# hby1320/pytorch_object_detection

Measured on AMD Instinct MI355X. Metric: images/sec HISFCOS-R50 640x640 inference, higher is better.
Workload: dtype f32

## Files before the change

### include/fcosdet.h

```cpp
#ifndef FCOSDET_H_
#define FCOSDET_H_

#include <stdint.h>

#ifdef __cplusplus
extern "C" {
#endif

#define FD_OK 0
#define FD_E_INVAL (-1)
#define FD_E_UNSUPPORTED (-2)
#define FD_E_LAUNCH (-3)

#define FD_MAX_SEG 8

#define FD_ACT_NONE 0
#define FD_ACT_RELU 1
#define FD_ACT_SILU 2
#define FD_ACT_EXP 3
#define FD_ACT_SIGMOID 4

typedef void* fd_stream_t;

typedef struct fd_segs {
// ... 229 lines not shown
                                     int32_t H, int32_t W, const float* mean3, const float* std3, fd_stream_t stream);
int32_t fd_jitter_l_sums(const uint8_t* const* images_dev, int32_t* recs_dev, uint64_t* sums_dev, int32_t N,
                         int64_t max_pixels, fd_stream_t stream);
int32_t fd_color_jitter_u8(const uint8_t* x, int32_t h, int32_t w, uint8_t* y, const int32_t* rec_dev, fd_stream_t stream);
int32_t fd_rotate_u8(const uint8_t* x, int32_t h, int32_t w, uint8_t* y, const int32_t* fixed6, fd_stream_t stream);

int64_t fd_groupnorm_workspace_bytes(const fd_segs* segs, int32_t G);
int32_t fd_groupnorm_act_nhwc(const float* x, int32_t x_cs, int32_t x_co, const float* gamma, const float* beta,
                              float* y, int32_t y_cs, int32_t y_co, int32_t C, int32_t G, float eps, int32_t act,
                              const fd_segs* segs, void* workspace, fd_stream_t stream);

int64_t fd_groupnorm_bwd_workspace_bytes(const fd_segs* segs, int32_t C);
int32_t fd_groupnorm_act_bwd_nhwc(const float* x, int32_t x_cs, int32_t x_co, const float* dy, int32_t dy_cs,
                                  int32_t dy_co, const float* gamma, const float* beta, float* dx, int32_t dx_cs,
                                  int32_t dx_co, float* dgamma, float* dbeta, int32_t C, int32_t G, float eps,
                                  int32_t act, const fd_segs* segs, const void* fwd_workspace, void* workspace,
                                  fd_stream_t stream);

int64_t fd_se_workspace_bytes(int32_t N, int32_t HW, int32_t C);
int32_t fd_se_scale_nhwc(const float* x, int32_t x_cs, int32_t x_co, const float* w1, const float* b1,
                         const float* w2, const float* b2, float* y, int32_t y_cs, int32_t y_co, int32_t N,
                         int32_t HW, int32_t C, int32_t Cr, void* workspace, fd_stream_t stream);

int64_t fd_se_bwd_workspace_bytes(int32_t N, int32_t HW, int32_t C);
int32_t fd_se_scale_bwd_nhwc(const float* x, int32_t x_cs, int32_t x_co, const float* dy, int32_t dy_cs, int32_t dy_co,
                             const float* w1, const float* b1, const float* w2, const float* b2, float* dx, int32_t dx_cs,
                             int32_t dx_co, float* dw1, float* db1, float* dw2, float* db2, int32_t N, int32_t HW, int32_t C,
                             int32_t Cr, const void* fwd_workspace, void* workspace, fd_stream_t stream);

int32_t fd_act_nhwc(const float* x, int32_t x_cs, int32_t x_co, float* y, int32_t y_cs, int32_t y_co, int64_t rows, int32_t C,
                    int32_t act, float param, fd_stream_t stream);
int32_t fd_act_bwd_nhwc(const float* x, int32_t x_cs, int32_t x_co, const float* dy, int32_t dy_cs, int32_t dy_co, float* dx,
                        int32_t dx_cs, int32_t dx_co, int64_t rows, int32_t C, int32_t act, float param, fd_stream_t stream);
int32_t fd_act_bwd_nhwc_h(const void* x, int32_t x_cs, int32_t x_co, const void* dy, int32_t dy_cs, int32_t dy_co, void* dx,
                          int32_t dx_cs, int32_t dx_co, int64_t rows, int32_t C, int32_t act, float param, fd_stream_t stream);

int32_t fd_maxpool_bwd_nhwc(const float* x, int32_t x_cs, int32_t x_co, const float* dy, int32_t dy_cs, int32_t dy_co, float* dx,
                            int32_t dx_cs, int32_t dx_co, int32_t N, int32_t H, int32_t W, int32_t C, int32_t k, int32_t s,
                            int32_t pad, fd_stream_t stream);
int32_t fd_upsample2x_bwd_nhwc(const float* dy, int32_t dy_cs, int32_t dy_co, float* dx, int32_t dx_cs, int32_t dx_co, int32_t N,
                               int32_t H, int32_t W, int32_t C, fd_stream_t stream);

int32_t fd_groupnorm_from_rowstats(const float* rowstats, int32_t C, int32_t G, float eps, const float* gamma, const float* beta,
                                   const fd_segs* segs, void* workspace, float* coef, fd_stream_t stream);
int32_t fd_groupnorm_apply_nhwc(const float* x, int32_t x_cs, int32_t x_co, const float* gamma, const float* beta, float* y,
                                int32_t y_cs, int32_t y_co, int32_t C, int32_t G, float eps, int32_t act, const fd_segs* segs,
// ... 114 lines not shown
```

### pytorch_object_detection_amd/_lib.py

```python
from __future__ import annotations

import ctypes as C
import os

FD_MAX_SEG = 8
ACT_NONE, ACT_RELU, ACT_SILU, ACT_EXP, ACT_SIGMOID = 0, 1, 2, 3, 4
CONV_GENERIC, CONV_STEM = 0, 1
PREC_F32, PREC_F16X3, PREC_F16 = 0, 1, 2
TILES = {1: (128, 128), 2: (128, 64), 3: (64, 128), 4: (64, 64), 5: (128, 32), 6: (128, 96),
         7: (128, 128), 8: (128, 64), 9: (64, 128),
         10: (256, 128), 11: (256, 128),
         12: (128, 96),
         13: (128, 128),
         15: (64, 64)}
PATCH_TILE = 13
WAVE_TILE = 15
WINO_TILE = 14
WINO4_TILE = 16
NARROW_TILE = 17
F16K64_TILE = 18

_HERE = os.path.dirname(os.path.abspath(__file__))
LIB_PATH = os.environ.get("FD_LIB") or os.path.join(_HERE, "csrc", "libfcosdet_hip.so")

# ... 125 lines not shown
    "fd_resize_u8": (_I, [_P, _I, _I, _P, _I, _I, _P]),
    "fd_resize_collate_u8_nhwc4": (_I, [_P, _P, _P, _P, _I, _I, _I, C.POINTER(_F), C.POINTER(_F), _P]),
    "fd_boxes_scale_batch": (_I, [_P, _P, _P, _I, _I, _I, _I, _P]),
    "fd_augment_resize_collate_u8": (_I, [_P, _P, _P, _I, _I, _I, C.POINTER(_F), C.POINTER(_F), _P]),
    "fd_jitter_l_sums": (_I, [_P, _P, _P, _I, _L, _P]),
    "fd_color_jitter_u8": (_I, [_P, _I, _I, _P, _P, _P]),
    "fd_rotate_u8": (_I, [_P, _I, _I, _P, C.POINTER(_I), _P]),
    "fd_dwconv_dilated_wgrad_workspace_bytes": (_L, [C.POINTER(Segs), _I, _I]),
    "fd_dwconv_dilated_bwd_weight_nhwc": (_I, [_P, _I, _I, _P, _I, _I, _P, _I, _I, _I, _P, _I, C.POINTER(Segs), _P, _P]),
    "fd_dwconv3x3_wgrad_workspace_bytes": (_L, [C.POINTER(Segs), _I]),
    "fd_dwconv3x3_bwd_weight_nhwc": (_I, [_P, _I, _I, _P, _I, _I, _P, _I, _P, _I, C.POINTER(Segs), _P, _P]),
    "fd_groupnorm_workspace_bytes": (_L, [C.POINTER(Segs), _I]),
    "fd_groupnorm_act_nhwc": (_I, [_P, _I, _I, _P, _P, _P, _I, _I, _I, _I, _F, _I, C.POINTER(Segs), _P, _P]),
    "fd_groupnorm_from_rowstats": (_I, [_P, _I, _I, _F, _P, _P, C.POINTER(Segs), _P, _P, _P]),
    "fd_groupnorm_apply_nhwc": (_I, [_P, _I, _I, _P, _P, _P, _I, _I, _I, _I, _F, _I, C.POINTER(Segs), _P, _P]),
    "fd_groupnorm_stats_nhwc": (_I, [_P, _I, _I, _I, _I, _F, _P, _P, C.POINTER(Segs), _P, _P, _P]),
    "fd_coef_apply_nhwc": (_I, [_P, _I, _I, _P, _P, _I, _P, _I, _I, _I, _I, C.POINTER(Segs), _P]),
    "fd_dwconv3x3_gn_nhwc": (_I, [_P, _I, _I, _P, _P, _I, _P, _I, _I, _I, _P, _I, C.POINTER(Segs), _P]),
    "fd_groupnorm_bwd_workspace_bytes": (_L, [C.POINTER(Segs), _I]),
    "fd_groupnorm_act_bwd_nhwc": (_I, [_P, _I, _I, _P, _I, _I, _P, _P, _P, _I, _I, _P, _P, _I, _I, _F, _I, C.POINTER(Segs), _P, _P,
                                       _P]),
    "fd_se_workspace_bytes": (_L, [_I, _I, _I]),
    "fd_se_scale_nhwc": (_I, [_P, _I, _I, _P, _P, _P, _P, _P, _I, _I, _I, _I, _I, _I, _P, _P]),
    "fd_se_bwd_workspace_bytes": (_L, [_I, _I, _I]),
    "fd_se_scale_bwd_nhwc": (_I, [_P, _I, _I, _P, _I, _I, _P, _P, _P, _P, _P, _I, _I, _P, _P, _P, _P, _I, _I, _I, _I, _P, _P, _P]),
    "fd_act_nhwc": (_I, [_P, _I, _I, _P, _I, _I, _L, _I, _I, _F, _P]),
    "fd_act_bwd_nhwc": (_I, [_P, _I, _I, _P, _I, _I, _P, _I, _I, _L, _I, _I, _F, _P]),
    "fd_act_bwd_nhwc_h": (_I, [_P, _I, _I, _P, _I, _I, _P, _I, _I, _L, _I, _I, _F, _P]),
    "fd_maxpool_bwd_nhwc": (_I, [_P, _I, _I, _P, _I, _I, _P, _I, _I, _I, _I, _I, _I, _I, _I, _I, _P]),
    "fd_upsample2x_bwd_nhwc": (_I, [_P, _I, _I, _P, _I, _I, _I, _I, _I, _I, _P]),
    "fd_batchnorm_update_running": (_I, [_P, _L, _I, _F, _F, _P, _P, _P]),
    "fd_batchnorm_update_running_dev": (_I, [_P, _P, _I, _F, _F, _P, _P, _P]),
    "fd_batchnorm_sync_fwd_nhwc": (_I, [_P, _I, _I, _P, _P, _P, _I, _I, _L, _I, _F, _I, _I, _P, _D, _P, _P]),
    "fd_batchnorm_sync_bwd_nhwc": (_I, [_P, _I, _I, _P, _I, _I, _P, _P, _P, _I, _I, _P, _P, _L, _I, _F, _I, _I, _P, _D, _P, _P, _P]),
    "fd_fcos_decode": (_I, [_P, _I, _I, _P, _I, _I, _P, _I, _I, _I, C.POINTER(Segs), C.POINTER(_I), _P, _P, _P, _P]),
    "fd_topk_workspace_bytes": (_L, [_I, _I, _I]),
    "fd_fcos_topk": (_I, [_P, _P, _P, _I, _I, _I, _P, _P, _P, _P, _P, _P]),
    "fd_nms_workspace_bytes": (_L, [_I, _I]),
    "fd_batched_nms": (_I, [_P, _P, _P, _I, _I, _F, _D, _P, _P, _P, _P, _P, _P, _P]),
    "fd_box_nms_plus1": (_I, [_P, _P, _P, _I, _I, _F, _I, _P, _P, _P]),
    "fd_pairwise_iou": (_I, [_P, _P, _I, _I, _I, _P, _P]),
    "fd_clip_boxes": (_I, [_P, _L, _I, _I, _P]),
    "fd_pack_detections": (_I, [_P, _P, _P, _P, _I, _I, _P, _P]),
    "fd_unpack_detections": (_I, [_P, _I, _I, _P, _P, _P, _P, _P]),
    "fd_ltrb_iou_loss_fwd": (_I, [_P, _P, _P, _I, _I, _I, _P, _P, _P]),
    "fd_ltrb_iou_loss_bwd": (_I, [_P, _P, _P, _P, _I, _I, _I, _P, _P]),
# ... 39 lines not shown
```

### pytorch_object_detection_amd/csrc/fd_layers.hip

```cpp
#include "fd_common.h"

#define FD_GRID_CAP 16384

static inline unsigned grid_for(long work, int block) {
    long g = (work + block - 1) / block;
    if (g > FD_GRID_CAP) g = FD_GRID_CAP;
    if (g < 1) g = 1;
    return (unsigned)g;
}

__global__ __launch_bounds__(256) void nchw3_to_nhwc4_kernel(const float* __restrict__ x, float4* __restrict__ y,
                                                              int HW, long total) {
    for (long i = (long)blockIdx.x * 256 + threadIdx.x; i < total; i += (long)gridDim.x * 256) {
        int pi;
        const long n = fd_div(i, HW, pi);
        const long p = pi;
        const float* b = x + n * 3 * HW + p;
        y[i] = make_float4(b[0], b[HW], b[2 * (long)HW], 0.f);
    }
}

extern "C" int32_t fd_nchw3_to_nhwc4(const float* x, float* y, int32_t N, int32_t H, int32_t W, fd_stream_t stream) {
    FD_REQUIRE(x && y && N >= 1 && H >= 1 && W >= 1, FD_E_INVAL, "fd_nchw3_to_nhwc4: bad argument");
    FD_REQUIRE(((uintptr_t)y & 15) == 0, FD_E_INVAL, "fd_nchw3_to_nhwc4: y not 16-byte aligned");
// ... 332 lines not shown
__device__ __forceinline__ void seg_decode(const fd_segs& sg, long m, int& H, int& W, long& img_row0, int& h, int& w) {
    int s = 0;
#pragma unroll
    for (int t = 1; t < FD_MAX_SEG; ++t)
        if (t < sg.nseg && m >= sg.m_start[t]) s = t;
    H = sg.H[s]; W = sg.W[s];
    const long local = m - sg.m_start[s];
    const int hw = H * W;
    int rem;
    const long n = fd_div(local, hw, rem);
    h = rem / W; w = rem - h * W;
    img_row0 = sg.m_start[s] + n * hw;
}

struct StripTab {
    fd_segs s;
    long strip_start[FD_MAX_SEG + 1];
    int spr[FD_MAX_SEG];
};

__device__ __forceinline__ float dw_quad_xor1(float v) { return __builtin_bit_cast(float, __builtin_amdgcn_mov_dpp(__builtin_bit_cast(int, v), 0xB1, 0xF, 0xF, true)); }
__device__ __forceinline__ float dw_quad_xor2(float v) { return __builtin_bit_cast(float, __builtin_amdgcn_mov_dpp(__builtin_bit_cast(int, v), 0x4E, 0xF, 0xF, true)); }

template <int S, bool FUSE = false>
__global__ __launch_bounds__(256) void dwconv3x3_strip_kernel(const float* __restrict__ x, int x_cs, int x_co,
                                                               const float* __restrict__ wt, const float* __restrict__ scale,
                                                               const float* __restrict__ shift, float* __restrict__ y, int y_cs,
                                                               int y_co, int C, int act, StripTab tab, long total,
                                                               const float* __restrict__ in_coef = nullptr, int in_act = 0,
                                                               float* __restrict__ gn_stats = nullptr, int gn_G = 1) {
    const int C4 = C >> 2;
    for (long i = (long)blockIdx.x * 256 + threadIdx.x; i < total; i += (long)gridDim.x * 256) {
        int q;
        const long t = fd_div(i, C4, q);
        int s = 0;
#pragma unroll
        for (int k = 1; k < FD_MAX_SEG; ++k)
            if (k < tab.s.nseg && t >= tab.strip_start[k]) s = k;
        const int H = tab.s.H[s], W = tab.s.W[s], spr = tab.spr[s];
        const long local = t - tab.strip_start[s];
        const int per_img = H * spr;
        int rem;
        const long n = fd_div(local, per_img, rem);
        const int h = rem / spr, w0 = (rem - h * spr) * S;
        const long r0 = (long)tab.s.m_start[s] + n * H * W;
        float4 ca = make_float4(1.f, 1.f, 1.f, 1.f), cb = make_float4(0.f, 0.f, 0.f, 0.f);
        const float act_lo = (FUSE && in_act == FD_ACT_RELU) ? 0.f : -INFINITY;
        if (FUSE && in_coef) {
            const float* cp = in_coef + ((long)(s * tab.s.batch + (int)n) * 2) * C + 4 * q;
            ca = *reinterpret_cast<const float4*>(cp);
            cb = *reinterpret_cast<const float4*>(cp + C);
        }
        float4 acc[S];
#pragma unroll
        for (int j = 0; j < S; ++j) acc[j] = make_float4(0.f, 0.f, 0.f, 0.f);
#pragma unroll
        for (int r = 0; r < 3; ++r) {
            const int hi = h + r - 1;
            if ((unsigned)hi >= (unsigned)H) continue;
            float4 u[S + 2];
#pragma unroll
            for (int c = 0; c < S + 2; ++c) {
                const int wi = w0 + c - 1;
                u[c] = (unsigned)wi < (unsigned)W ? *reinterpret_cast<const float4*>(x + (r0 + (long)hi * W + wi) * x_cs + x_co + 4 * q)
                                                  : make_float4(0.f, 0.f, 0.f, 0.f);
            }
            if (FUSE && in_coef) {
#pragma unroll
                for (int c = 0; c < S + 2; ++c) {
                    float4 t = make_float4(fmaf(u[c].x, ca.x, cb.x), fmaf(u[c].y, ca.y, cb.y), fmaf(u[c].z, ca.z, cb.z), fmaf(u[c].w, ca.w, cb.w));
                    t.x = fmaxf(t.x, act_lo); t.y = fmaxf(t.y, act_lo); t.z = fmaxf(t.z, act_lo); t.w = fmaxf(t.w, act_lo);
                    if (in_act == FD_ACT_SILU) {
                        t.x *= __builtin_amdgcn_rcpf(1.0f + __expf(-t.x)); t.y *= __builtin_amdgcn_rcpf(1.0f + __expf(-t.y));
                        t.z *= __builtin_amdgcn_rcpf(1.0f + __expf(-t.z)); t.w *= __builtin_amdgcn_rcpf(1.0f + __expf(-t.w));
                    }
                    const bool inb = (unsigned)(w0 + c - 1) < (unsigned)W;
                    u[c] = inb ? t : make_float4(0.f, 0.f, 0.f, 0.f);
                }
            }
#pragma unroll
            for (int c = 0; c < 3; ++c) {
                const float4 k = *reinterpret_cast<const float4*>(wt + (r * 3 + c) * C + 4 * q);
#pragma unroll
                for (int j = 0; j < S; ++j) {
                    if ((unsigned)(w0 + j + c - 1) < (unsigned)W) {
                        acc[j].x = fmaf(u[j + c].x, k.x, acc[j].x); acc[j].y = fmaf(u[j + c].y, k.y, acc[j].y);
                        acc[j].z = fmaf(u[j + c].z, k.z, acc[j].z); acc[j].w = fmaf(u[j + c].w, k.w, acc[j].w);
                    }
                }
            }
        }
        float4 sc = make_float4(1.f, 1.f, 1.f, 1.f), sf = make_float4(0.f, 0.f, 0.f, 0.f);
        if (scale) sc = *reinterpret_cast<const float4*>(scale + 4 * q);
        if (shift) sf = *reinterpret_cast<const float4*>(shift + 4 * q);
#pragma unroll
        for (int j = 0; j < S; ++j) {
            if (w0 + j >= W) break;
            float4 o;
            o = fd_act4(make_float4(acc[j].x * sc.x + sf.x, acc[j].y * sc.y + sf.y, acc[j].z * sc.z + sf.z, acc[j].w * sc.w + sf.w), act, 0.f);
            const long mo = r0 + (long)h * W + w0 + j;
            *reinterpret_cast<float4*>(y + mo * y_cs + y_co + 4 * q) = o;
            if (FUSE && gn_stats) {
                float s1 = (o.x + o.y) + (o.z + o.w), s2 = (o.x * o.x + o.y * o.y) + (o.z * o.z + o.w * o.w);
                const int cgq = (C / gn_G) >> 2;
                if (cgq > 1) { s1 += dw_quad_xor1(s1); s2 += dw_quad_xor1(s2); }
                if (cgq > 2) { s1 += dw_quad_xor2(s1); s2 += dw_quad_xor2(s2); }
                if (cgq > 4) { s1 += __shfl_xor(s1, 4); s2 += __shfl_xor(s2, 4); }
                if ((q & (cgq - 1)) == 0) reinterpret_cast<float2*>(gn_stats)[mo * gn_G + (4 * q) / (C / gn_G)] = make_float2(s1, s2);
            }
        }
    }
}

extern "C" int32_t fd_dwconv3x3_nhwc(const float* x, int32_t x_cs, int32_t x_co, const float* w, const float* scale,
                                     const float* shift, float* y, int32_t y_cs, int32_t y_co, int32_t C, int32_t act,
                                     const fd_segs* segs, fd_stream_t stream) {
    FD_REQUIRE(fd_segs_ok(segs), FD_E_INVAL, "fd_dwconv3x3: bad segment table");
    FD_REQUIRE(view_ok(x, x_cs, x_co, C) && view_ok(y, y_cs, y_co, C) && w && ((uintptr_t)w & 15) == 0, FD_E_INVAL,
               "fd_dwconv3x3: channel views must be 4-aligned (C=%d)", C);
    StripTab tab; tab.s = *segs;
    const int S = (long)segs->m_start[segs->nseg] * (C / 4) >= (16L << 20) ? 8 : 4;
    long strips = 0;
    for (int s = 0; s < FD_MAX_SEG; ++s) {
        tab.strip_start[s] = strips;
        tab.spr[s] = s < segs->nseg ? (segs->W[s] + S - 1) / S : 1;
        if (s < segs->nseg) strips += (long)segs->batch * segs->H[s] * tab.spr[s];
    }
    tab.strip_start[FD_MAX_SEG] = strips;
    const long total = strips * (C / 4);
    if (S == 8)
        hipLaunchKernelGGL(dwconv3x3_strip_kernel<8>, dim3(grid_for(total, 256)), dim3(256), 0, (hipStream_t)stream, x, x_cs, x_co,
                           w, scale, shift, y, y_cs, y_co, C, act, tab, total);
    else
        hipLaunchKernelGGL(dwconv3x3_strip_kernel<4>, dim3(grid_for(total, 256)), dim3(256), 0, (hipStream_t)stream, x, x_cs, x_co,
                           w, scale, shift, y, y_cs, y_co, C, act, tab, total);
    FD_CHECK_LAUNCH("fd_dwconv3x3_nhwc");
    return FD_OK;
}

extern "C" int32_t fd_dwconv3x3_gn_nhwc(const float* x, int32_t x_cs, int32_t x_co, const float* w, const float* in_coef, int32_t in_act,
                                        float* y, int32_t y_cs, int32_t y_co, int32_t C, float* gn_stats, int32_t gn_groups,
                                        const fd_segs* segs, fd_stream_t stream) {
    FD_REQUIRE(fd_segs_ok(segs), FD_E_INVAL, "fd_dwconv3x3_gn: bad segment table");
    FD_REQUIRE(view_ok(x, x_cs, x_co, C) && view_ok(y, y_cs, y_co, C) && w && ((uintptr_t)w & 15) == 0, FD_E_INVAL,
               "fd_dwconv3x3_gn: channel views must be 4-aligned (C=%d)", C);
    FD_REQUIRE(!in_coef || (((uintptr_t)in_coef & 15) == 0 && (in_act == FD_ACT_NONE || in_act == FD_ACT_RELU || in_act == FD_ACT_SILU)), FD_E_INVAL,
               "fd_dwconv3x3_gn: in_coef must be 16-byte aligned, in_act in {NONE, RELU, SILU}");
    if (gn_stats) {
        const int cg = gn_groups >= 1 && C % gn_groups == 0 ? C / gn_groups : 0;
        FD_REQUIRE(cg >= 4 && cg % 4 == 0 && 32 % cg == 0 && (((C / 4) % 64 == 0) || (64 % (C / 4) == 0)) && ((uintptr_t)gn_stats & 7) == 0,
                   FD_E_UNSUPPORTED, "fd_dwconv3x3_gn: gn_stats needs 4 | C / groups | 32 and C / 4 a multiple or divisor of 64 (C=%d groups=%d)", C, gn_groups);
    }
    StripTab tab; tab.s = *segs;
    const int S = (long)segs->m_start[segs->nseg] * (C / 4) >= (16L << 20) ? 8 : 4;
    long strips = 0;
    for (int s = 0; s < FD_MAX_SEG; ++s) {
        tab.strip_start[s] = strips;
        tab.spr[s] = s < segs->nseg ? (segs->W[s] + S - 1) / S : 1;
        if (s < segs->nseg) strips += (long)segs->batch * segs->H[s] * tab.spr[s];
    }
    tab.strip_start[FD_MAX_SEG] = strips;
    const long total = strips * (C / 4);
    if (S == 8)
        hipLaunchKernelGGL((dwconv3x3_strip_kernel<8, true>), dim3(grid_for(total, 256)), dim3(256), 0, (hipStream_t)stream, x, x_cs, x_co,
                           w, (const float*)nullptr, (const float*)nullptr, y, y_cs, y_co, C, FD_ACT_NONE, tab, total, in_coef, in_act, gn_stats, gn_groups);
    else
        hipLaunchKernelGGL((dwconv3x3_strip_kernel<4, true>), dim3(grid_for(total, 256)), dim3(256), 0, (hipStream_t)stream, x, x_cs, x_co,
                           w, (const float*)nullptr, (const float*)nullptr, y, y_cs, y_co, C, FD_ACT_NONE, tab, total, in_coef, in_act, gn_stats, gn_groups);
    FD_CHECK_LAUNCH("fd_dwconv3x3_gn_nhwc");
    return FD_OK;
}

__global__ __launch_bounds__(256) void dwconv_dilated_kernel(const float* __restrict__ x, int x_cs, int x_co, const float* __restrict__ wt,
                                                              const float* __restrict__ scale, const float* __restrict__ shift,
                                                              float* __restrict__ y, int y_cs, int y_co, int C, int K, int dil, int act,
                                                              SegTab tab, long total) {
    const int C4 = C >> 2;
    for (long i = (long)blockIdx.x * 256 + threadIdx.x; i < total; i += (long)gridDim.x * 256) {
        int q;
        const long m = fd_div(i, C4, q);
        int H, W, h, w;
        long row0;
        seg_decode(tab.s, m, H, W, row0, h, w);
        const int half = (K - 1) / 2;
        float4 acc = make_float4(0.f, 0.f, 0.f, 0.f);
        for (int r = 0; r < K; ++r) {
            const int hi = h + (r - half) * dil;
            if ((unsigned)hi >= (unsigned)H) continue;
            for (int c = 0; c < K; ++c) {
                const int wi = w + (c - half) * dil;
                if ((unsigned)wi >= (unsigned)W) continue;
// ... 803 lines not shown
        int j = 0;
        for (; j + 4 <= Cr; j += 4) {
            a0 = fmaf(wr[j], s_h[j], a0); a1 = fmaf(wr[j + 1], s_h[j + 1], a1);
            a2 = fmaf(wr[j + 2], s_h[j + 2], a2); a3 = fmaf(wr[j + 3], s_h[j + 3], a3);
        }
        for (; j < Cr; ++j) a0 = fmaf(wr[j], s_h[j], a0);
        gate[(long)n * C + c] = fd_sigmoid((a0 + a1) + (a2 + a3));
    }
}

__global__ __launch_bounds__(256) void se_scale_kernel(const float* __restrict__ x, int x_cs, int x_co,
                                                        const float* __restrict__ gate, float* __restrict__ y, int y_cs,
                                                        int y_co, int HW, int C4, long total) {
    for (long i = (long)blockIdx.x * 256 + threadIdx.x; i < total; i += (long)gridDim.x * 256) {
        int q;
        const long m = fd_div(i, C4, q);
        int hw_rem_; const long n = fd_div(m, HW, hw_rem_);
        const float4 v = *reinterpret_cast<const float4*>(x + m * x_cs + x_co + 4 * q);
        const float4 g = *reinterpret_cast<const float4*>(gate + n * C4 * 4 + 4 * q);
        *reinterpret_cast<float4*>(y + m * y_cs + y_co + 4 * q) = make_float4(v.x * g.x, v.y * g.y, v.z * g.z, v.w * g.w);
    }
}

extern "C" int64_t fd_se_workspace_bytes(int32_t N, int32_t HW, int32_t C) {
    if (N < 1 || HW < 1 || C < 1) return -1;
    return (int64_t)N * SE_MAXCHUNK * C * (int64_t)sizeof(double) + (int64_t)N * C * (int64_t)sizeof(float);
}

extern "C" int32_t fd_se_scale_nhwc(const float* x, int32_t x_cs, int32_t x_co, const float* w1, const float* b1,
                                    const float* w2, const float* b2, float* y, int32_t y_cs, int32_t y_co, int32_t N,
                                    int32_t HW, int32_t C, int32_t Cr, void* workspace, fd_stream_t stream) {
    FD_REQUIRE(view_ok(x, x_cs, x_co, C) && (!y || view_ok(y, y_cs, y_co, C)) && w1 && w2 && workspace, FD_E_INVAL,
               "fd_se_scale: bad pointer / channel view (C=%d)", C);
    FD_REQUIRE(N >= 1 && N <= 65535 && HW >= 1 && Cr >= 1 && Cr <= SE_MAXCR && C <= SE_MAXC, FD_E_UNSUPPORTED,
               "fd_se_scale: C=%d Cr=%d unsupported (C <= %d, Cr <= %d)", C, Cr, SE_MAXC, SE_MAXCR);
    FD_REQUIRE(((uintptr_t)workspace & 15) == 0, FD_E_INVAL, "fd_se_scale: workspace not 16-byte aligned");
    double* part = (double*)workspace;
    float* gate = (float*)((char*)workspace + (size_t)N * SE_MAXCHUNK * C * sizeof(double));
    const int nchunk = min(SE_MAXCHUNK, (HW + 63) / 64);
    int QW = 1;
    while (QW < 64 && QW < C / 4) QW <<= 1;
    hipLaunchKernelGGL(se_gap_kernel, dim3(nchunk, N, (C / 4 + QW - 1) / QW), dim3(256), 0, (hipStream_t)stream, x, x_cs, x_co, HW, C,
                       nchunk, QW, part);
    FD_CHECK_LAUNCH("fd_se_scale (gap)");
    hipLaunchKernelGGL(se_fc_kernel, dim3(N, (C + 255) / 256), dim3(256), 0, (hipStream_t)stream, (const double*)part, nchunk, HW, C, Cr, w1,
                       b1, w2, b2, gate);
    FD_CHECK_LAUNCH("fd_se_scale (fc)");
    if (!y) return FD_OK;
    const long total = (long)N * HW * (C / 4);
    hipLaunchKernelGGL(se_scale_kernel, dim3(grid_for(total, 256)), dim3(256), 0, (hipStream_t)stream, x, x_cs, x_co,
                       (const float*)gate, y, y_cs, y_co, HW, C / 4, total);
    FD_CHECK_LAUNCH("fd_se_scale (scale)");
    return FD_OK;
}


__global__ __launch_bounds__(256) void se_pool_reduce_kernel(const float* __restrict__ pool, int T, int tpc, int C, double* __restrict__ part) {
    const int n = blockIdx.y, k = blockIdx.z;
    const int t0 = k * tpc, t1 = min(T, t0 + tpc);
    for (int c = blockIdx.x * 256 + threadIdx.x; c < C; c += gridDim.x * 256) {
        const float* p = pool + (size_t)n * T * C + c;
        double a0 = 0, a1 = 0, a2 = 0, a3 = 0;
        int t = t0;
        for (; t + 4 <= t1; t += 4) { a0 += p[(size_t)t * C]; a1 += p[(size_t)(t + 1) * C]; a2 += p[(size_t)(t + 2) * C]; a3 += p[(size_t)(t + 3) * C]; }
        for (; t < t1; ++t) a0 += p[(size_t)t * C];
        part[((size_t)n * SE_MAXCHUNK + k) * C + c] = (a0 + a1) + (a2 + a3);
    }
}

extern "C" int32_t fd_se_gate_from_pool(const float* pool, int32_t T, const float* w1, const float* b1, const float* w2, const float* b2, int32_t N, int32_t HW,
                                        int32_t C, int32_t Cr, void* workspace, fd_stream_t stream) {
    FD_REQUIRE(pool && w1 && w2 && workspace && T >= 1 && C % 4 == 0, FD_E_INVAL, "fd_se_gate_from_pool: bad arguments (C=%d T=%d)", C, T);
    FD_REQUIRE(N >= 1 && N <= 65535 && HW >= 1 && Cr >= 1 && Cr <= SE_MAXCR && C <= SE_MAXC, FD_E_UNSUPPORTED,
               "fd_se_gate_from_pool: C=%d Cr=%d unsupported (C <= %d, Cr <= %d)", C, Cr, SE_MAXC, SE_MAXCR);
    FD_REQUIRE(((uintptr_t)workspace & 15) == 0, FD_E_INVAL, "fd_se_gate_from_pool: workspace not 16-byte aligned");
// ... 280 lines not shown
```

### pytorch_object_detection_amd/engine.py

```python
from __future__ import annotations

from typing import Callable, Dict, List, Optional, Sequence, Tuple

import torch

from . import ops
from . import _lib
from ._lib import ACT_EXP, ACT_NONE, ACT_RELU, ACT_SILU, FdError, Segs
from .ops import Rows


import os as _os

CONV_PRECISION = _os.environ.get("FD_CONV_PRECISION", "f32")
AUTOTUNE = True
GN_FUSED = _os.environ.get("FD_GN_FUSED", "1") != "0"
B2B_MIN_ROWS = 64 * 1024
B2B_LAYERS = "1"


class PRows(Rows):
    __slots__ = ("_flat",)


# ... 481 lines not shown
    half = blk.conv1.weight.shape[0]
    N, HW = segs.batch, segs.H[0] * segs.W[0]
    cat1 = pool.get(M, 2 * half)
    cat2 = pool.get(M, 2 * half)
    s1, t1 = ops.fold_bn(_dev(blk.bn1.weight, dev), _dev(blk.bn1.bias, dev), _dev(blk.bn1.running_mean, dev),
                         _dev(blk.bn1.running_var, dev), blk.bn1.eps, _dev(blk.conv1.bias, dev) if blk.conv1.bias is not None else None)
    bias2 = _dev(blk.conv2.bias, dev) if blk.conv2.bias is not None else torch.zeros(half, device=dev)
    w12 = torch.cat([blk.conv2.weight.detach(), blk.conv1.weight.detach()], 0)
    fold = (torch.cat([torch.ones(half, device=dev), s1]).contiguous(), torch.cat([bias2, t1]).contiguous())
    add_conv(plan, name + ".conv1+2", x, segs, blk.conv1, cat2, weight=w12, Cout=2 * half, act=ACT_SILU, act_c0=half, fold=fold)
    x1 = cat2.slice(half, half)
    wd = ops.pack_dw_weight(_dev(blk.conv1_1.weight, dev))
    sc, sf = ops.fold_bn(_dev(blk.bn2.weight, dev), _dev(blk.bn2.bias, dev), _dev(blk.bn2.running_mean, dev),
                         _dev(blk.bn2.running_var, dev), blk.bn2.eps)
    u = cat1.slice(0, half)
    se = blk.conv1_2.excitation
    w1 = _dev(se[0].weight, dev).reshape(se[0].weight.shape[0], -1).contiguous()
    b1 = _dev(se[0].bias, dev)
    w2 = _dev(se[2].weight, dev).reshape(se[2].weight.shape[0], -1).contiguous()
    b2 = _dev(se[2].bias, dev)
    ws = ops.se_workspace(N, HW, half, dev)
    v = cat1.slice(half, half)
    cr = w1.shape[0]
    plan.add(name + ".conv1_1", lambda: ops.dwconv3x3(x1, wd, u, segs, sc, sf, ACT_RELU))
    plan.add(name + ".conv1_2", lambda: ops.se_scale(x1, w1, b1, w2, b2, v, N, HW, cr, ws))
    plan.keep += [wd, sc, sf, w1, b1, w2, b2, ws]
    add_conv(plan, name + ".conv3", cat1, segs, blk.conv3, cat2.slice(half, half), bn=blk.bn3, act=ACT_RELU)
    w4 = blk.conv4.weight.detach()
    add_conv(plan, name + ".conv4", cat2, segs, blk.conv4, out, bn=blk.bn4, act=ACT_SILU,
             weight=torch.cat([w4[:, half:], w4[:, :half]], 1))
    pool.put(cat1); pool.put(cat2)


def build_his_fpn(plan: Plan, fpn, feats):
    pool = plan.pool
    (c3, s3), (c4, s4), (c5, s5) = feats
    B = s3.batch
    F = fpn.tf1.weight.shape[0]
    h5, w5 = s5.H[0], s5.W[0]
    hw = [(s3.H[0], s3.W[0]), (s4.H[0], s4.W[0]), (h5, w5), (h5 // 2, w5 // 2), (h5 // 4, w5 // 4)]
    if hw[4][0] < 1 or hw[4][1] < 1:
        raise FdError("HISFCOS FPN: input too small for the stride-128 level")
    if (s4.H[0], s4.W[0]) != (2 * h5, 2 * w5) or (s3.H[0], s3.W[0]) != (4 * h5, 4 * w5):
        raise FdError("HISFCOS FPN: H and W must be multiples of 32 (x2 upsample-adds must line up, HISFcos.py:155-165)")
    pyr_segs = Segs.make(B, hw)
    pyr = pool.get(pyr_segs.rows, F)

    lv = [Rows(pyr.buf[pyr_segs.m_start[i]:pyr_segs.m_start[i + 1]]) for i in range(5)]
# ... 387 lines not shown
```

### pytorch_object_detection_amd/ops.py

```python
from __future__ import annotations

import ctypes as C
import enum
import json
import math
import os
import re
from typing import Callable, List, NamedTuple, Optional, Sequence, Tuple

import numpy as np
import torch

from . import _lib
from ._lib import ACT_EXP, ACT_NONE, ACT_RELU, ACT_SIGMOID, ACT_SILU, ConvParams, FdError, Segs, check


CONV_LOG = None
LAUNCHES = [0]


def _stream() -> int:
    LAUNCHES[0] += 1
    return torch.cuda.current_stream().cuda_stream

# ... 1227 lines not shown
    if n < 0:
        raise FdError("fd_groupnorm_bwd_workspace_bytes: bad arguments")
    ws = torch.empty(n // 8, dtype=torch.float64, device=dev)
    dgamma = torch.empty(x.C, dtype=torch.float32, device=dev)
    dbeta = torch.empty(x.C, dtype=torch.float32, device=dev)
    check(_lib.lib().fd_groupnorm_act_bwd_nhwc(x.ptr, x.cs, x.co, dy.ptr, dy.cs, dy.co, gamma.data_ptr(), beta.data_ptr(),
                                               dx.ptr, dx.cs, dx.co, dgamma.data_ptr(), dbeta.data_ptr(), x.C, G, eps, act,
                                               C.byref(segs), fwd_ws.data_ptr(), ws.data_ptr(), _stream()),
          "fd_groupnorm_act_bwd_nhwc")
    return dgamma, dbeta


def se_workspace(N: int, HW: int, C_: int, device) -> torch.Tensor:
    n = _lib.lib().fd_se_workspace_bytes(N, HW, C_)
    return torch.empty((n + 7) // 8, dtype=torch.float64, device=device)


def se_scale(x: Rows, w1, b1, w2, b2, y: Rows, N: int, HW: int, Cr: int, ws: torch.Tensor) -> None:
    check(_lib.lib().fd_se_scale_nhwc(x.ptr, x.cs, x.co, w1.data_ptr(), b1.data_ptr() if b1 is not None else None,
                                      w2.data_ptr(), b2.data_ptr() if b2 is not None else None, y.ptr, y.cs, y.co, N, HW,
                                      x.C, Cr, ws.data_ptr(), _stream()), "fd_se_scale_nhwc")


def se_gate(x: Rows, w1, b1, w2, b2, N: int, HW: int, Cr: int, ws: torch.Tensor) -> torch.Tensor:
    check(_lib.lib().fd_se_scale_nhwc(x.ptr, x.cs, x.co, w1.data_ptr(), b1.data_ptr() if b1 is not None else None,
                                      w2.data_ptr(), b2.data_ptr() if b2 is not None else None, None, 0, 0, N, HW,
                                      x.C, Cr, ws.data_ptr(), _stream()), "fd_se_scale_nhwc")
    return se_gate_view(ws, N, HW, x.C)


def se_gate_view(ws: torch.Tensor, N: int, HW: int, C_: int) -> torch.Tensor:
    nbytes = _lib.lib().fd_se_workspace_bytes(N, HW, C_)
    return ws.view(torch.float32)[nbytes // 4 - N * C_: nbytes // 4].view(N, C_)


def se_scale_bwd(x: Rows, dy: Rows, w1, b1, w2, b2, dx: Rows, N: int, HW: int, Cr: int, fwd_ws: torch.Tensor):
    dev = x.buf.device
    Cc = x.C
    n = _lib.lib().fd_se_bwd_workspace_bytes(N, HW, Cc)
    ws = torch.empty((n + 7) // 8, dtype=torch.float64, device=dev)
    dw1 = torch.empty(Cr, Cc, dtype=torch.float32, device=dev)
    db1 = torch.empty(Cr, dtype=torch.float32, device=dev)
    dw2 = torch.empty(Cc, Cr, dtype=torch.float32, device=dev)
    db2 = torch.empty(Cc, dtype=torch.float32, device=dev)
    check(_lib.lib().fd_se_scale_bwd_nhwc(x.ptr, x.cs, x.co, dy.ptr, dy.cs, dy.co, w1.data_ptr(), b1.data_ptr() if b1 is not None else None,
                                          w2.data_ptr(), b2.data_ptr() if b2 is not None else None, dx.ptr, dx.cs, dx.co, dw1.data_ptr(),
# ... 421 lines not shown
```

Baseline: 1427.

## Fuse SE channel scaling into depthwise 3x3 strip kernel and add row-blocking

Adds a combined depthwise-conv + squeeze-excitation entry point: the SE gate is computed first, then the depthwise strip kernel writes both the conv output and the gated copy of its input. This avoids a separate pass that re-reads the input just to scale it. The strip kernel also gains a row-blocking parameter R, so each thread computes several output rows and reuses loaded input rows and register-cached weights. Strip width for large tensors drops from 8 to 4. These changes add register pressure and a new size-based tiling heuristic that affects every depthwise call.

```diff
diff --git a/include/fcosdet.h b/include/fcosdet.h
--- a/include/fcosdet.h
+++ b/include/fcosdet.h
@@ -275,6 +275,11 @@
                          const float* w2, const float* b2, float* y, int32_t y_cs, int32_t y_co, int32_t N,
                          int32_t HW, int32_t C, int32_t Cr, void* workspace, fd_stream_t stream);
 
+int32_t fd_dwconv3x3_se_nhwc(const float* x, int32_t x_cs, int32_t x_co, const float* w, const float* scale, const float* shift,
+                             int32_t act, const float* w1, const float* b1, const float* w2, const float* b2, int32_t Cr,
+                             float* u, int32_t u_cs, int32_t u_co, float* v, int32_t v_cs, int32_t v_co, int32_t C,
+                             const fd_segs* segs, void* workspace, fd_stream_t stream);
+
 int64_t fd_se_bwd_workspace_bytes(int32_t N, int32_t HW, int32_t C);
 int32_t fd_se_scale_bwd_nhwc(const float* x, int32_t x_cs, int32_t x_co, const float* dy, int32_t dy_cs, int32_t dy_co,
                              const float* w1, const float* b1, const float* w2, const float* b2, float* dx, int32_t dx_cs,
diff --git a/pytorch_object_detection_amd/_lib.py b/pytorch_object_detection_amd/_lib.py
--- a/pytorch_object_detection_amd/_lib.py
+++ b/pytorch_object_detection_amd/_lib.py
@@ -171,6 +171,7 @@
                                        _P]),
     "fd_se_workspace_bytes": (_L, [_I, _I, _I]),
     "fd_se_scale_nhwc": (_I, [_P, _I, _I, _P, _P, _P, _P, _P, _I, _I, _I, _I, _I, _I, _P, _P]),
+    "fd_dwconv3x3_se_nhwc": (_I, [_P, _I, _I, _P, _P, _P, _I, _P, _P, _P, _P, _I, _P, _I, _I, _P, _I, _I, _I, C.POINTER(Segs), _P, _P]),
     "fd_se_bwd_workspace_bytes": (_L, [_I, _I, _I]),
     "fd_se_scale_bwd_nhwc": (_I, [_P, _I, _I, _P, _I, _I, _P, _P, _P, _P, _P, _I, _I, _P, _P, _P, _P, _I, _I, _I, _I, _P, _P, _P]),
     "fd_act_nhwc": (_I, [_P, _I, _I, _P, _I, _I, _L, _I, _I, _F, _P]),
diff --git a/pytorch_object_detection_amd/csrc/fd_layers.hip b/pytorch_object_detection_amd/csrc/fd_layers.hip
--- a/pytorch_object_detection_amd/csrc/fd_layers.hip
+++ b/pytorch_object_detection_amd/csrc/fd_layers.hip
@@ -378,13 +378,15 @@
 __device__ __forceinline__ float dw_quad_xor1(float v) { return __builtin_bit_cast(float, __builtin_amdgcn_mov_dpp(__builtin_bit_cast(int, v), 0xB1, 0xF, 0xF, true)); }
 __device__ __forceinline__ float dw_quad_xor2(float v) { return __builtin_bit_cast(float, __builtin_amdgcn_mov_dpp(__builtin_bit_cast(int, v), 0x4E, 0xF, 0xF, true)); }
 
-template <int S, bool FUSE = false>
+template <int S, int R = 1, bool FUSE = false, bool SE = false>
 __global__ __launch_bounds__(256) void dwconv3x3_strip_kernel(const float* __restrict__ x, int x_cs, int x_co,
                                                                const float* __restrict__ wt, const float* __restrict__ scale,
                                                                const float* __restrict__ shift, float* __restrict__ y, int y_cs,
                                                                int y_co, int C, int act, StripTab tab, long total,
                                                                const float* __restrict__ in_coef = nullptr, int in_act = 0,
-                                                               float* __restrict__ gn_stats = nullptr, int gn_G = 1) {
+                                                               float* __restrict__ gn_stats = nullptr, int gn_G = 1,
+                                                               const float* __restrict__ se_gate = nullptr, float* __restrict__ v = nullptr,
+                                                               int v_cs = 0, int v_co = 0) {
     const int C4 = C >> 2;
     for (long i = (long)blockIdx.x * 256 + threadIdx.x; i < total; i += (long)gridDim.x * 256) {
         int q;
@@ -395,10 +397,10 @@
             if (k < tab.s.nseg && t >= tab.strip_start[k]) s = k;
         const int H = tab.s.H[s], W = tab.s.W[s], spr = tab.spr[s];
         const long local = t - tab.strip_start[s];
-        const int per_img = H * spr;
+        const int per_img = ((H + R - 1) / R) * spr;
         int rem;
         const long n = fd_div(local, per_img, rem);
-        const int h = rem / spr, w0 = (rem - h * spr) * S;
+        const int rg = rem / spr, w0 = (rem - rg * spr) * S, h0 = rg * R;
         const long r0 = (long)tab.s.m_start[s] + n * H * W;
         float4 ca = make_float4(1.f, 1.f, 1.f, 1.f), cb = make_float4(0.f, 0.f, 0.f, 0.f);
         const float act_lo = (FUSE && in_act == FD_ACT_RELU) ? 0.f : -INFINITY;
@@ -407,65 +409,124 @@
             ca = *reinterpret_cast<const float4*>(cp);
             cb = *reinterpret_cast<const float4*>(cp + C);
         }
-        float4 acc[S];
-#pragma unroll
-        for (int j = 0; j < S; ++j) acc[j] = make_float4(0.f, 0.f, 0.f, 0.f);
-#pragma unroll
-        for (int r = 0; r < 3; ++r) {
-            const int hi = h + r - 1;
-            if ((unsigned)hi >= (unsigned)H) continue;
-            float4 u[S + 2];
-#pragma unroll
-            for (int c = 0; c < S + 2; ++c) {
-                const int wi = w0 + c - 1;
-                u[c] = (unsigned)wi < (unsigned)W ? *reinterpret_cast<const float4*>(x + (r0 + (long)hi * W + wi) * x_cs + x_co + 4 * q)
-                                                  : make_float4(0.f, 0.f, 0.f, 0.f);
-            }
-            if (FUSE && in_coef) {
+        float4 kr[R > 1 ? 9 : 1];
+        float4 sc = make_float4(1.f, 1.f, 1.f, 1.f), sf = make_float4(0.f, 0.f, 0.f, 0.f);
+        if (R > 1) {
+#pragma unroll
+            for (int e = 0; e < 9; ++e) kr[e] = *reinterpret_cast<const float4*>(wt + e * C + 4 * q);
+            if (scale) sc = *reinterpret_cast<const float4*>(scale + 4 * q);
+            if (shift) sf = *reinterpret_cast<const float4*>(shift + 4 * q);
+        }
+        float4 g = make_float4(1.f, 1.f, 1.f, 1.f);
+        if (SE) g = *reinterpret_cast<const float4*>(se_gate + n * C + 4 * q);
+        float4 acc[R][S];
+#pragma unroll
+        for (int o = 0; o < R; ++o)
+#pragma unroll
+            for (int j = 0; j < S; ++j) acc[o][j] = make_float4(0.f, 0.f, 0.f, 0.f);
+#pragma unroll
+        for (int it = 0; it < R + 2; ++it) {
+            const int hi = h0 + it - 1;
+            if ((unsigned)hi < (unsigned)H) {
+                float4 u[S + 2];
 #pragma unroll
                 for (int c = 0; c < S + 2; ++c) {
-                    float4 t = make_float4(fmaf(u[c].x, ca.x, cb.x), fmaf(u[c].y, ca.y, cb.y), fmaf(u[c].z, ca.z, cb.z), fmaf(u[c].w, ca.w, cb.w));
-                    t.x = fmaxf(t.x, act_lo); t.y = fmaxf(t.y, act_lo); t.z = fmaxf(t.z, act_lo); t.w = fmaxf(t.w, act_lo);
-                    if (in_act == FD_ACT_SILU) {
-                        t.x *= __builtin_amdgcn_rcpf(1.0f + __expf(-t.x)); t.y *= __builtin_amdgcn_rcpf(1.0f + __expf(-t.y));
-                        t.z *= __builtin_amdgcn_rcpf(1.0f + __expf(-t.z)); t.w *= __builtin_amdgcn_rcpf(1.0f + __expf(-t.w));
+                    const int wi = w0 + c - 1;
+                    u[c] = (unsigned)wi < (unsigned)W ? *reinterpret_cast<const float4*>(x + (r0 + (long)hi * W + wi) * x_cs + x_co + 4 * q)
+                                                      : make_float4(0.f, 0.f, 0.f, 0.f);
+                }
+                if (FUSE && in_coef) {
+#pragma unroll
+                    for (int c = 0; c < S + 2; ++c) {
+                        float4 t = make_float4(fmaf(u[c].x, ca.x, cb.x), fmaf(u[c].y, ca.y, cb.y), fmaf(u[c].z, ca.z, cb.z), fmaf(u[c].w, ca.w, cb.w));
+                        t.x = fmaxf(t.x, act_lo); t.y = fmaxf(t.y, act_lo); t.z = fmaxf(t.z, act_lo); t.w = fmaxf(t.w, act_lo);
+                        if (in_act == FD_ACT_SILU) {
+                            t.x *= __builtin_amdgcn_rcpf(1.0f + __expf(-t.x)); t.y *= __builtin_amdgcn_rcpf(1.0f + __expf(-t.y));
+                            t.z *= __builtin_amdgcn_rcpf(1.0f + __expf(-t.z)); t.w *= __builtin_amdgcn_rcpf(1.0f + __expf(-t.w));
+                        }
+                        const bool inb = (unsigned)(w0 + c - 1) < (unsigned)W;
+                        u[c] = inb ? t : make_float4(0.f, 0.f, 0.f, 0.f);
                     }
-                    const bool inb = (unsigned)(w0 + c - 1) < (unsigned)W;
-                    u[c] = inb ? t : make_float4(0.f, 0.f, 0.f, 0.f);
                 }
-            }
-#pragma unroll
-            for (int c = 0; c < 3; ++c) {
-                const float4 k = *reinterpret_cast<const float4*>(wt + (r * 3 + c) * C + 4 * q);
-#pragma unroll
-                for (int j = 0; j < S; ++j) {
-                    if ((unsigned)(w0 + j + c - 1) < (unsigned)W) {
-                        acc[j].x = fmaf(u[j + c].x, k.x, acc[j].x); acc[j].y = fmaf(u[j + c].y, k.y, acc[j].y);
-                        acc[j].z = fmaf(u[j + c].z, k.z, acc[j].z); acc[j].w = fmaf(u[j + c].w, k.w, acc[j].w);
+                if (SE && it >= 1 && it <= R) {
+#pragma unroll
+                    for (int j = 0; j < S; ++j) {
+                        if (w0 + j >= W) break;
+                        *reinterpret_cast<float4*>(v + (r0 + (long)hi * W + w0 + j) * v_cs + v_co + 4 * q) =
+                            make_float4(u[j + 1].x * g.x, u[j + 1].y * g.y, u[j + 1].z * g.z, u[j + 1].w * g.w);
+                    }
+                }
+#pragma unroll
+                for (int r = 0; r < 3; ++r) {
+                    const int o = it - r;
+                    if (o < 0 || o >= R) continue;
+#pragma unroll
+                    for (int c = 0; c < 3; ++c) {
+                        const float4 k = R > 1 ? kr[R > 1 ? r * 3 + c : 0] : *reinterpret_cast<const float4*>(wt + (r * 3 + c) * C + 4 * q);
+#pragma unroll
+                        for (int j = 0; j < S; ++j) {
+                            if ((unsigned)(w0 + j + c - 1) < (unsigned)W) {
+                                acc[o][j].x = fmaf(u[j + c].x, k.x, acc[o][j].x); acc[o][j].y = fmaf(u[j + c].y, k.y, acc[o][j].y);
+                                acc[o][j].z = fmaf(u[j + c].z, k.z, acc[o][j].z); acc[o][j].w = fmaf(u[j + c].w, k.w, acc[o][j].w);
+                            }
+                        }
                     }
                 }
             }
-        }
-        float4 sc = make_float4(1.f, 1.f, 1.f, 1.f), sf = make_float4(0.f, 0.f, 0.f, 0.f);
-        if (scale) sc = *reinterpret_cast<const float4*>(scale + 4 * q);
-        if (shift) sf = *reinterpret_cast<const float4*>(shift + 4 * q);
-#pragma unroll
-        for (int j = 0; j < S; ++j) {
-            if (w0 + j >= W) break;
-            float4 o;
-            o = fd_act4(make_float4(acc[j].x * sc.x + sf.x, acc[j].y * sc.y + sf.y, acc[j].z * sc.z + sf.z, acc[j].w * sc.w + sf.w), act, 0.f);
-            const long mo = r0 + (long)h * W + w0 + j;
-            *reinterpret_cast<float4*>(y + mo * y_cs + y_co + 4 * q) = o;
-            if (FUSE && gn_stats) {
-                float s1 = (o.x + o.y) + (o.z + o.w), s2 = (o.x * o.x + o.y * o.y) + (o.z * o.z + o.w * o.w);
-                const int cgq = (C / gn_G) >> 2;
-                if (cgq > 1) { s1 += dw_quad_xor1(s1); s2 += dw_quad_xor1(s2); }
-                if (cgq > 2) { s1 += dw_quad_xor2(s1); s2 += dw_quad_xor2(s2); }
-                if (cgq > 4) { s1 += __shfl_xor(s1, 4); s2 += __shfl_xor(s2, 4); }
-                if ((q & (cgq - 1)) == 0) reinterpret_cast<float2*>(gn_stats)[mo * gn_G + (4 * q) / (C / gn_G)] = make_float2(s1, s2);
+            if (it < 2) continue;
+            const int ro = it - 2, h = h0 + ro;
+            if (h >= H) continue;
+            if (R == 1) {
+                if (scale) sc = *reinterpret_cast<const float4*>(scale + 4 * q);
+                if (shift) sf = *reinterpret_cast<const float4*>(shift + 4 * q);
             }
-        }
-    }
+#pragma unroll
+            for (int j = 0; j < S; ++j) {
+                if (w0 + j >= W) break;
+                float4 o;
+                o = fd_act4(make_float4(acc[ro][j].x * sc.x + sf.x, acc[ro][j].y * sc.y + sf.y, acc[ro][j].z * sc.z + sf.z, acc[ro][j].w * sc.w + sf.w), act, 0.f);
+                const long mo = r0 + (long)h * W + w0 + j;
+                *reinterpret_cast<float4*>(y + mo * y_cs + y_co + 4 * q) = o;
+                if (FUSE && gn_stats) {
+                    float s1 = (o.x + o.y) + (o.z + o.w), s2 = (o.x * o.x + o.y * o.y) + (o.z * o.z + o.w * o.w);
+                    const int cgq = (C / gn_G) >> 2;
+                    if (cgq > 1) { s1 += dw_quad_xor1(s1); s2 += dw_quad_xor1(s2); }
+                    if (cgq > 2) { s1 += dw_quad_xor2(s1); s2 += dw_quad_xor2(s2); }
+                    if (cgq > 4) { s1 += __shfl_xor(s1, 4); s2 += __shfl_xor(s2, 4); }
+                    if ((q & (cgq - 1)) == 0) reinterpret_cast<float2*>(gn_stats)[mo * gn_G + (4 * q) / (C / gn_G)] = make_float2(s1, s2);
+                }
+            }
+        }
+    }
+}
+
+struct DwShape { int S, R; };
+static DwShape dw_strip_shape(const fd_segs* segs, int C) {
+    const long px4 = (long)segs->m_start[segs->nseg] * (C / 4);
+    DwShape d;
+    d.S = 4;
+    d.R = px4 >= (2L << 20) ? 4 : px4 >= (768L << 10) ? 2 : 1;
+    return d;
+}
+
+static long dw_strip_tab(StripTab& tab, const fd_segs* segs, DwShape d) {
+    tab.s = *segs;
+    long strips = 0;
+    for (int s = 0; s < FD_MAX_SEG; ++s) {
+        tab.strip_start[s] = strips;
+        tab.spr[s] = s < segs->nseg ? (segs->W[s] + d.S - 1) / d.S : 1;
+        if (s < segs->nseg) strips += (long)segs->batch * ((segs->H[s] + d.R - 1) / d.R) * tab.spr[s];
+    }
+    tab.strip_start[FD_MAX_SEG] = strips;
+    return strips;
+}
+
+template <bool FUSE, bool SE, typename... Args>
+static void dw_strip_launch(DwShape d, long total, hipStream_t st, Args... args) {
+    const dim3 grid(grid_for(total, 256)), block(256);
+    if (d.R == 4) hipLaunchKernelGGL((dwconv3x3_strip_kernel<4, 4, FUSE, SE>), grid, block, 0, st, args...);
+    else if (d.R == 2) hipLaunchKernelGGL((dwconv3x3_strip_kernel<4, 2, FUSE, SE>), grid, block, 0, st, args...);
+    else hipLaunchKernelGGL((dwconv3x3_strip_kernel<4, 1, FUSE, SE>), grid, block, 0, st, args...);
 }
 
 extern "C" int32_t fd_dwconv3x3_nhwc(const float* x, int32_t x_cs, int32_t x_co, const float* w, const float* scale,
@@ -474,22 +535,11 @@
     FD_REQUIRE(fd_segs_ok(segs), FD_E_INVAL, "fd_dwconv3x3: bad segment table");
     FD_REQUIRE(view_ok(x, x_cs, x_co, C) && view_ok(y, y_cs, y_co, C) && w && ((uintptr_t)w & 15) == 0, FD_E_INVAL,
                "fd_dwconv3x3: channel views must be 4-aligned (C=%d)", C);
-    StripTab tab; tab.s = *segs;
-    const int S = (long)segs->m_start[segs->nseg] * (C / 4) >= (16L << 20) ? 8 : 4;
-    long strips = 0;
-    for (int s = 0; s < FD_MAX_SEG; ++s) {
-        tab.strip_start[s] = strips;
-        tab.spr[s] = s < segs->nseg ? (segs->W[s] + S - 1) / S : 1;
-        if (s < segs->nseg) strips += (long)segs->batch * segs->H[s] * tab.spr[s];
-    }
-    tab.strip_start[FD_MAX_SEG] = strips;
-    const long total = strips * (C / 4);
-    if (S == 8)
-        hipLaunchKernelGGL(dwconv3x3_strip_kernel<8>, dim3(grid_for(total, 256)), dim3(256), 0, (hipStream_t)stream, x, x_cs, x_co,
-                           w, scale, shift, y, y_cs, y_co, C, act, tab, total);
-    else
-        hipLaunchKernelGGL(dwconv3x3_strip_kernel<4>, dim3(grid_for(total, 256)), dim3(256), 0, (hipStream_t)stream, x, x_cs, x_co,
-                           w, scale, shift, y, y_cs, y_co, C, act, tab, total);
+    StripTab tab;
+    const DwShape d = dw_strip_shape(segs, C);
+    const long total = dw_strip_tab(tab, segs, d) * (C / 4);
+    dw_strip_launch<false, false>(d, total, (hipStream_t)stream, x, x_cs, x_co, w, scale, shift, y, y_cs, y_co, C, act, tab, total,
+                                  (const float*)nullptr, 0, (float*)nullptr, 1, (const float*)nullptr, (float*)nullptr, 0, 0);
     FD_CHECK_LAUNCH("fd_dwconv3x3_nhwc");
     return FD_OK;
 }
@@ -507,22 +557,11 @@
         FD_REQUIRE(cg >= 4 && cg % 4 == 0 && 32 % cg == 0 && (((C / 4) % 64 == 0) || (64 % (C / 4) == 0)) && ((uintptr_t)gn_stats & 7) == 0,
                    FD_E_UNSUPPORTED, "fd_dwconv3x3_gn: gn_stats needs 4 | C / groups | 32 and C / 4 a multiple or divisor of 64 (C=%d groups=%d)", C, gn_groups);
     }
-    StripTab tab; tab.s = *segs;
-    const int S = (long)segs->m_start[segs->nseg] * (C / 4) >= (16L << 20) ? 8 : 4;
-    long strips = 0;
-    for (int s = 0; s < FD_MAX_SEG; ++s) {
-        tab.strip_start[s] = strips;
-        tab.spr[s] = s < segs->nseg ? (segs->W[s] + S - 1) / S : 1;
-        if (s < segs->nseg) strips += (long)segs->batch * segs->H[s] * tab.spr[s];
-    }
-    tab.strip_start[FD_MAX_SEG] = strips;
-    const long total = strips * (C / 4);
-    if (S == 8)
-        hipLaunchKernelGGL((dwconv3x3_strip_kernel<8, true>), dim3(grid_for(total, 256)), dim3(256), 0, (hipStream_t)stream, x, x_cs, x_co,
-                           w, (const float*)nullptr, (const float*)nullptr, y, y_cs, y_co, C, FD_ACT_NONE, tab, total, in_coef, in_act, gn_stats, gn_groups);
-    else
-        hipLaunchKernelGGL((dwconv3x3_strip_kernel<4, true>), dim3(grid_for(total, 256)), dim3(256), 0, (hipStream_t)stream, x, x_cs, x_co,
-                           w, (const float*)nullptr, (const float*)nullptr, y, y_cs, y_co, C, FD_ACT_NONE, tab, total, in_coef, in_act, gn_stats, gn_groups);
+    StripTab tab;
+    const DwShape d = dw_strip_shape(segs, C);
+    const long total = dw_strip_tab(tab, segs, d) * (C / 4);
+    dw_strip_launch<true, false>(d, total, (hipStream_t)stream, x, x_cs, x_co, w, (const float*)nullptr, (const float*)nullptr, y, y_cs, y_co, C,
+                                 (int)FD_ACT_NONE, tab, total, in_coef, in_act, gn_stats, gn_groups, (const float*)nullptr, (float*)nullptr, 0, 0);
     FD_CHECK_LAUNCH("fd_dwconv3x3_gn_nhwc");
     return FD_OK;
 }
@@ -1372,6 +1411,18 @@
     }
 }
 
+static const float* se_gates_launch(const float* x, int x_cs, int x_co, const float* w1, const float* b1, const float* w2, const float* b2,
+                                    int N, int HW, int C, int Cr, void* workspace, hipStream_t st) {
+    double* part = (double*)workspace;
+    float* gate = (float*)((char*)workspace + (size_t)N * SE_MAXCHUNK * C * sizeof(double));
+    const int nchunk = min(SE_MAXCHUNK, (HW + 63) / 64);
+    int QW = 1;
+    while (QW < 64 && QW < C / 4) QW <<= 1;
+    hipLaunchKernelGGL(se_gap_kernel, dim3(nchunk, N, (C / 4 + QW - 1) / QW), dim3(256), 0, st, x, x_cs, x_co, HW, C, nchunk, QW, part);
+    hipLaunchKernelGGL(se_fc_kernel, dim3(N, (C + 255) / 256), dim3(256), 0, st, (const double*)part, nchunk, HW, C, Cr, w1, b1, w2, b2, gate);
+    return gate;
+}
+
 extern "C" int64_t fd_se_workspace_bytes(int32_t N, int32_t HW, int32_t C) {
     if (N < 1 || HW < 1 || C < 1) return -1;
     return (int64_t)N * SE_MAXCHUNK * C * (int64_t)sizeof(double) + (int64_t)N * C * (int64_t)sizeof(float);
@@ -1385,22 +1436,37 @@
     FD_REQUIRE(N >= 1 && N <= 65535 && HW >= 1 && Cr >= 1 && Cr <= SE_MAXCR && C <= SE_MAXC, FD_E_UNSUPPORTED,
                "fd_se_scale: C=%d Cr=%d unsupported (C <= %d, Cr <= %d)", C, Cr, SE_MAXC, SE_MAXCR);
     FD_REQUIRE(((uintptr_t)workspace & 15) == 0, FD_E_INVAL, "fd_se_scale: workspace not 16-byte aligned");
-    double* part = (double*)workspace;
-    float* gate = (float*)((char*)workspace + (size_t)N * SE_MAXCHUNK * C * sizeof(double));
-    const int nchunk = min(SE_MAXCHUNK, (HW + 63) / 64);
-    int QW = 1;
-    while (QW < 64 && QW < C / 4) QW <<= 1;
-    hipLaunchKernelGGL(se_gap_kernel, dim3(nchunk, N, (C / 4 + QW - 1) / QW), dim3(256), 0, (hipStream_t)stream, x, x_cs, x_co, HW, C,
-                       nchunk, QW, part);
-    FD_CHECK_LAUNCH("fd_se_scale (gap)");
-    hipLaunchKernelGGL(se_fc_kernel, dim3(N, (C + 255) / 256), dim3(256), 0, (hipStream_t)stream, (const double*)part, nchunk, HW, C, Cr, w1,
-                       b1, w2, b2, gate);
-    FD_CHECK_LAUNCH("fd_se_scale (fc)");
+    const float* gate = se_gates_launch(x, x_cs, x_co, w1, b1, w2, b2, N, HW, C, Cr, workspace, (hipStream_t)stream);
+    FD_CHECK_LAUNCH("fd_se_scale (gap, fc)");
     if (!y) return FD_OK;
     const long total = (long)N * HW * (C / 4);
     hipLaunchKernelGGL(se_scale_kernel, dim3(grid_for(total, 256)), dim3(256), 0, (hipStream_t)stream, x, x_cs, x_co,
-                       (const float*)gate, y, y_cs, y_co, HW, C / 4, total);
+                       gate, y, y_cs, y_co, HW, C / 4, total);
     FD_CHECK_LAUNCH("fd_se_scale (scale)");
+    return FD_OK;
+}
+
+
+extern "C" int32_t fd_dwconv3x3_se_nhwc(const float* x, int32_t x_cs, int32_t x_co, const float* w, const float* scale, const float* shift,
+                                        int32_t act, const float* w1, const float* b1, const float* w2, const float* b2, int32_t Cr,
+                                        float* u, int32_t u_cs, int32_t u_co, float* v, int32_t v_cs, int32_t v_co, int32_t C,
+                                        const fd_segs* segs, void* workspace, fd_stream_t stream) {
+    FD_REQUIRE(fd_segs_ok(segs), FD_E_INVAL, "fd_dwconv3x3_se: bad segment table");
+    FD_REQUIRE(segs->nseg == 1, FD_E_UNSUPPORTED, "fd_dwconv3x3_se: one level only (nseg=%d)", segs->nseg);
+    FD_REQUIRE(view_ok(x, x_cs, x_co, C) && view_ok(u, u_cs, u_co, C) && view_ok(v, v_cs, v_co, C) && w && ((uintptr_t)w & 15) == 0 && w1 && w2 &&
+               workspace, FD_E_INVAL, "fd_dwconv3x3_se: bad pointer / channel views must be 4-aligned (C=%d)", C);
+    const int N = segs->batch, HW = segs->H[0] * segs->W[0];
+    FD_REQUIRE(N <= 65535 && Cr >= 1 && Cr <= SE_MAXCR && C <= SE_MAXC, FD_E_UNSUPPORTED,
+               "fd_dwconv3x3_se: C=%d Cr=%d unsupported (C <= %d, Cr <= %d)", C, Cr, SE_MAXC, SE_MAXCR);
+    FD_REQUIRE(((uintptr_t)workspace & 15) == 0, FD_E_INVAL, "fd_dwconv3x3_se: workspace not 16-byte aligned");
+    const float* gate = se_gates_launch(x, x_cs, x_co, w1, b1, w2, b2, N, HW, C, Cr, workspace, (hipStream_t)stream);
+    FD_CHECK_LAUNCH("fd_dwconv3x3_se (gap, fc)");
+    StripTab tab;
+    const DwShape d = dw_strip_shape(segs, C);
+    const long total = dw_strip_tab(tab, segs, d) * (C / 4);
+    dw_strip_launch<false, true>(d, total, (hipStream_t)stream, x, x_cs, x_co, w, scale, shift, u, u_cs, u_co, C, act, tab, total,
+                                 (const float*)nullptr, 0, (float*)nullptr, 1, gate, v, v_cs, v_co);
+    FD_CHECK_LAUNCH("fd_dwconv3x3_se (strip)");
     return FD_OK;
 }
 
diff --git a/pytorch_object_detection_amd/engine.py b/pytorch_object_detection_amd/engine.py
--- a/pytorch_object_detection_amd/engine.py
+++ b/pytorch_object_detection_amd/engine.py
@@ -527,8 +527,7 @@
     ws = ops.se_workspace(N, HW, half, dev)
     v = cat1.slice(half, half)
     cr = w1.shape[0]
-    plan.add(name + ".conv1_1", lambda: ops.dwconv3x3(x1, wd, u, segs, sc, sf, ACT_RELU))
-    plan.add(name + ".conv1_2", lambda: ops.se_scale(x1, w1, b1, w2, b2, v, N, HW, cr, ws))
+    plan.add(name + ".conv1_1+1_2", lambda: ops.dwconv3x3_se(x1, wd, sc, sf, ACT_RELU, w1, b1, w2, b2, cr, u, v, segs, ws))
     plan.keep += [wd, sc, sf, w1, b1, w2, b2, ws]
     add_conv(plan, name + ".conv3", cat1, segs, blk.conv3, cat2.slice(half, half), bn=blk.bn3, act=ACT_RELU)
     w4 = blk.conv4.weight.detach()
diff --git a/pytorch_object_detection_amd/ops.py b/pytorch_object_detection_amd/ops.py
--- a/pytorch_object_detection_amd/ops.py
+++ b/pytorch_object_detection_amd/ops.py
@@ -1273,6 +1273,16 @@
                                       x.C, Cr, ws.data_ptr(), _stream()), "fd_se_scale_nhwc")
 
 
+def dwconv3x3_se(x: Rows, w9c: torch.Tensor, scale, shift, act: int, w1, b1, w2, b2, Cr: int, u: Rows, v: Rows, segs: Segs,
+                 ws: torch.Tensor) -> None:
+    _need_gpu(w9c, w1, w2, ws)
+    check(_lib.lib().fd_dwconv3x3_se_nhwc(x.ptr, x.cs, x.co, w9c.data_ptr(), scale.data_ptr() if scale is not None else None,
+                                          shift.data_ptr() if shift is not None else None, act, w1.data_ptr(),
+                                          b1.data_ptr() if b1 is not None else None, w2.data_ptr(), b2.data_ptr() if b2 is not None else None,
+                                          Cr, u.ptr, u.cs, u.co, v.ptr, v.cs, v.co, x.C, C.byref(segs), ws.data_ptr(), _stream()),
+          "fd_dwconv3x3_se_nhwc")
+
+
 def se_gate(x: Rows, w1, b1, w2, b2, N: int, HW: int, Cr: int, ws: torch.Tensor) -> torch.Tensor:
     check(_lib.lib().fd_se_scale_nhwc(x.ptr, x.cs, x.co, w1.data_ptr(), b1.data_ptr() if b1 is not None else None,
                                       w2.data_ptr(), b2.data_ptr() if b2 is not None else None, None, 0, 0, N, HW,
```

After: 1428 (median of 2 runs). About the same (+0.1%).
